# AntreasAntoniou/HowToTrainYourMAMLPytorch

Measured on AMD Instinct MI355X. Metric: meta-tasks/sec, higher is better.
Workload: dtype bf16; 1 GPU; model=maml++_miniimagenet_5w1s, global_batch=128, tasks_per_gpu=128, ways=5, shots=1, targets=15, filters=48, inner_steps=5, msl=True, parallelism=task-dp1

## Files before the change

howtotrainyourmamlpytorch_amd/ops/hip/dconv.hip:

```cpp

#include "common.h"
#include <torch/extension.h>
#include <ATen/cuda/CUDAContext.h>

using namespace maml355;

using bf16 = __hip_bfloat16;
typedef __attribute__((__vector_size__(8 * sizeof(short)))) short bf16x8;

template <int FT>
__global__ __launch_bounds__(256)
void dconv_fwd_kernel(const bf16* __restrict__ X, const float* __restrict__ W,
                      const float* __restrict__ bias, bf16* __restrict__ Y,
                      int T, int NB, int H, int Wd, int C,
                      int Ho, int Wo, int pad) {
  const int t = blockIdx.y;
  __shared__ float wl[9 * 8 * FT];
  const float* Wt = W + (long)t * FT * C * 9;
  for (int i = threadIdx.x; i < FT * C * 9; i += blockDim.x) {
    const int kyx = i % 9;
    const int c = (i / 9) % C;
    const int f = i / (9 * C);
    wl[(kyx * C + c) * FT + f] = Wt[i];
  }
  __syncthreads();

  const long Mtot = (long)NB * Ho * Wo;
  const bf16* Xt = X + (long)t * NB * H * Wd * C;
  bf16* Yt = Y + (long)t * Mtot * FT;
  const float* bt = bias ? bias + (long)t * FT : nullptr;

  for (long m = (long)blockIdx.x * blockDim.x + threadIdx.x; m < Mtot;
       m += (long)blockDim.x * gridDim.x) {
    const int wo = (int)(m % Wo);
    const int ho = (int)((m / Wo) % Ho);
    const int n = (int)(m / ((long)Wo * Ho));
    float acc[FT];
#pragma unroll
    for (int f = 0; f < FT; ++f) acc[f] = bt ? bt[f] : 0.f;
    for (int ky = 0; ky < 3; ++ky) {
      const int h = ho + ky - pad;
      if (h < 0 || h >= H) continue;
      for (int kx = 0; kx < 3; ++kx) {
        const int w = wo + kx - pad;
        if (w < 0 || w >= Wd) continue;
        const short* xrow = (const short*)Xt + (((long)n * H + h) * Wd + w) * C;
        for (int c = 0; c < C; ++c) {
          const float xv = __bfloat162float(
              __hip_bfloat16(__hip_bfloat16_raw{(unsigned short)xrow[c]}));
          const float* wp = &wl[((ky * 3 + kx) * C + c) * FT];
#pragma unroll
          for (int f = 0; f < FT; ++f) acc[f] = fmaf(xv, wp[f], acc[f]);
        }
      }
    }
#pragma unroll
    for (int f8 = 0; f8 < FT / 8; ++f8) {
      bf16x8 v;
#pragma unroll
      for (int j = 0; j < 8; ++j)
        v[j] = (short)__bfloat16_as_short(__float2bfloat16(acc[f8 * 8 + j]));
      *(bf16x8*)&((short*)Yt)[m * FT + f8 * 8] = v;
    }
  }
}

template <int CT, bool DET>
__global__ __launch_bounds__(256)
void dconv_wgrad_kernel(const bf16* __restrict__ dY, const bf16* __restrict__ X,
                        float* __restrict__ dWacc, float* __restrict__ dBacc,
                        int T, int NB, int H, int Wd, int Ho, int Wo, int F,
                        int pad, long chunk) {
  const int t = blockIdx.y;
  const long Mtot = (long)NB * Ho * Wo;
  const int wave = threadIdx.x / WAVE;
  const int lane = threadIdx.x % WAVE;
  const int nwaves = blockDim.x / WAVE;
  const long c0 = blockIdx.x * chunk + wave * (chunk / nwaves);
  const long c1 = min(c0 + chunk / nwaves, Mtot);

  const bf16* Xt = X + (long)t * NB * H * Wd * CT;
  const short* dYt = (const short*)dY + (long)t * Mtot * F;

  float acc[9 * CT];
#pragma unroll
  for (int i = 0; i < 9 * CT; ++i) acc[i] = 0.f;
  float db = 0.f;

  if (c0 < Mtot) {
    int wo = (int)(c0 % Wo);
    int ho = (int)((c0 / Wo) % Ho);
    int n = (int)(c0 / ((long)Wo * Ho));
    for (long m = c0; m < c1; ++m) {
      const float dyv =
          (lane < F)
              ? __bfloat162float(__hip_bfloat16(
                    __hip_bfloat16_raw{(unsigned short)dYt[m * F + lane]}))
              : 0.f;
      db += dyv;
#pragma unroll
      for (int ky = 0; ky < 3; ++ky) {
        const int h = ho + ky - pad;
        if (h < 0 || h >= H) continue;
#pragma unroll
        for (int kx = 0; kx < 3; ++kx) {
          const int w = wo + kx - pad;
          if (w < 0 || w >= Wd) continue;
          const short* xrow =
              (const short*)Xt + (((long)n * H + h) * Wd + w) * CT;
#pragma unroll
          for (int c = 0; c < CT; ++c) {
            const float xv = __bfloat162float(__hip_bfloat16(
                __hip_bfloat16_raw{(unsigned short)xrow[c]}));
            acc[(ky * 3 + kx) * CT + c] = fmaf(dyv, xv, acc[(ky * 3 + kx) * CT + c]);
          }
        }
      }
      if (++wo == Wo) {
        wo = 0;
        if (++ho == Ho) { ho = 0; ++n; }
      }
    }
  }

  float* dWt = DET ? dWacc + ((long)t * gridDim.x + blockIdx.x) * 9 * CT * F
                   : dWacc + (long)t * 9 * CT * F;
  {
    __shared__ float red[256];
#pragma unroll
    for (int i = 0; i < 9 * CT; ++i) {
      red[threadIdx.x] = acc[i];
      __syncthreads();
      if (wave == 0 && lane < F) {
        float s = 0.f;
        for (int wv = 0; wv < nwaves; ++wv) s += red[wv * WAVE + lane];
        if (DET) {
          dWt[(long)i * F + lane] = s;
        } else {
          atomicAdd(&dWt[(long)i * F + lane], s);
        }
      }
      __syncthreads();
    }
  }
  if (dBacc != nullptr) {
    __shared__ float dbl[256];
    dbl[threadIdx.x] = db;
    __syncthreads();
    if (wave == 0 && lane < F) {
      float s = 0.f;
      for (int wv = 0; wv < nwaves; ++wv) s += dbl[wv * WAVE + lane];
      if (DET) {
        dBacc[((long)t * gridDim.x + blockIdx.x) * F + lane] = s;
      } else {
        atomicAdd(&dBacc[(long)t * F + lane], s);
      }
    }
  }
}

__global__ void dconv_finalize_kernel(const float* __restrict__ acc,
                                      float* __restrict__ dw,
                                      int T, int F, int C, int nslices) {
  const long total = (long)T * F * C * 9;
  const long ssz = (long)9 * C * F;
  for (long i = (long)blockIdx.x * blockDim.x + threadIdx.x; i < total;
       i += grid_stride()) {
    long r = i;
    const int kx = (int)(r % 3); r /= 3;
    const int ky = (int)(r % 3); r /= 3;
    const int c = (int)(r % C); r /= C;
    const int f = (int)(r % F); r /= F;
    const long t = r;
    const long e = ((long)(ky * 3 + kx) * C + c) * F + f;
    float v = 0.f;
    for (int s = 0; s < nslices; ++s) v += acc[(t * nslices + s) * ssz + e];
    dw[i] = v;
  }
}

torch::Tensor dconv_fwd(torch::Tensor x, torch::Tensor w,
                        c10::optional<torch::Tensor> bias, long pad,
                        long Ho, long Wo) {
  TORCH_CHECK(x.is_cuda() && x.dim() == 5 && x.is_contiguous());
  TORCH_CHECK(x.scalar_type() == torch::kBFloat16);
  const int T = (int)x.size(0), NB = (int)x.size(1), H = (int)x.size(2),
            W = (int)x.size(3), C = (int)x.size(4);
  const int F = (int)w.size(1);
  TORCH_CHECK(C <= 8 && (F == 16 || F == 32 || F == 48 || F == 64),
              "dconv_fwd needs C<=8 and F in {16,32,48,64}");
  auto wc = w.contiguous().to(torch::kFloat32);
  auto y = torch::empty({T, NB, Ho, Wo, F}, x.options());
  const float* bptr = nullptr;
  torch::Tensor bc;
  if (bias.has_value()) {
    bc = bias->contiguous().to(torch::kFloat32);
    bptr = bc.data_ptr<float>();
  }
  const long Mtot = (long)NB * Ho * Wo;
  const int blocks = (int)std::min<long>((Mtot + 255) / 256, 4096);
  auto stream = at::cuda::getCurrentCUDAStream();
#define LAUNCH_DFWD(FT)                                                        \
  hipLaunchKernelGGL((dconv_fwd_kernel<FT>), dim3(blocks, T), dim3(256), 0,    \
                     stream.stream(),                                          \
                     reinterpret_cast<const bf16*>(x.data_ptr()),              \
                     wc.data_ptr<float>(), bptr,                               \
                     reinterpret_cast<bf16*>(y.data_ptr()),                    \
                     T, NB, H, W, C, (int)Ho, (int)Wo, (int)pad)
  switch (F) {
    case 16: LAUNCH_DFWD(16); break;
    case 32: LAUNCH_DFWD(32); break;
    case 48: LAUNCH_DFWD(48); break;
    default: LAUNCH_DFWD(64); break;
  }
#undef LAUNCH_DFWD
  return y;
}

std::vector<torch::Tensor> dconv_wgrad(torch::Tensor dy, torch::Tensor x,
                                       long pad, bool with_bias) {
  TORCH_CHECK(dy.is_cuda() && x.is_cuda());
  auto dyc = dy.contiguous();
  auto xc = x.contiguous();
  const int T = (int)x.size(0), NB = (int)x.size(1), H = (int)x.size(2),
            W = (int)x.size(3), C = (int)x.size(4);
  const int Ho = (int)dy.size(2), Wo = (int)dy.size(3), F = (int)dy.size(4);
  TORCH_CHECK(C <= 8 && F <= 64, "dconv_wgrad needs C<=8, F<=64");
  const char* det_env = getenv("MAML355_DETERMINISTIC");
  const bool det = det_env && det_env[0] == '1';
  const long Mtot = (long)NB * Ho * Wo;
  long gridx = std::max<long>(1, 2048 / std::max(1, T));
  long chunk = (Mtot + gridx - 1) / gridx;
  chunk = std::max<long>(((chunk + 3) / 4) * 4, 4);
  gridx = (Mtot + chunk - 1) / chunk;
  const int nslices = det ? (int)gridx : 1;
  auto acc = torch::zeros({T, nslices, 9 * C, F},
                          x.options().dtype(torch::kFloat32));
  auto dbacc = torch::zeros({T, nslices, F},
                            x.options().dtype(torch::kFloat32));
  auto stream = at::cuda::getCurrentCUDAStream();
#define LAUNCH_DWG(CT, DET_)                                                   \
  hipLaunchKernelGGL((dconv_wgrad_kernel<CT, DET_>), dim3((unsigned)gridx, T), \
                     dim3(256), 0, stream.stream(),                            \
                     reinterpret_cast<const bf16*>(dyc.data_ptr()),            \
                     reinterpret_cast<const bf16*>(xc.data_ptr()),             \
                     acc.data_ptr<float>(),                                    \
                     with_bias ? dbacc.data_ptr<float>() : nullptr,            \
                     T, NB, H, W, Ho, Wo, F, (int)pad, chunk)
#define LAUNCH_DWG_DET(CT)                                                     \
  do { if (det) LAUNCH_DWG(CT, true); else LAUNCH_DWG(CT, false); } while (0)
  switch (C) {
    case 1: LAUNCH_DWG_DET(1); break;
    case 2: LAUNCH_DWG_DET(2); break;
    case 3: LAUNCH_DWG_DET(3); break;
    case 4: LAUNCH_DWG_DET(4); break;
    default: LAUNCH_DWG_DET(8); break;
  }
#undef LAUNCH_DWG
#undef LAUNCH_DWG_DET
  auto dw = torch::empty({T, F, C, 3, 3}, x.options().dtype(torch::kFloat32));
  const long total = (long)T * F * C * 9;
  const int fb = (int)std::min<long>((total + 255) / 256, 4096);
  hipLaunchKernelGGL(dconv_finalize_kernel, dim3(fb), dim3(256), 0,
                     stream.stream(), acc.data_ptr<float>(),
                     dw.data_ptr<float>(), T, F, C, nslices);
  auto db = nslices == 1 ? dbacc.select(1, 0).contiguous() : dbacc.sum(1);
  return {dw, db};
}
```

howtotrainyourmamlpytorch_amd/ops/hip/tconv.hip:

```cpp

#include "common.h"
#include <torch/extension.h>
#include <ATen/cuda/CUDAContext.h>

using namespace maml355;

using bf16 = __hip_bfloat16;
typedef __attribute__((__vector_size__(8 * sizeof(short)))) short bf16x8;
typedef __attribute__((__vector_size__(4 * sizeof(float)))) float f32x4;

DEVINL int swz64(int row, int col) {
  return (row * 64 + col) ^ ((row & 7) << 3);
}
DEVINL int swz128(int row, int col) {
  return (row * 128 + col) ^ ((row & 7) << 3);
}

__global__ void repack_weight_kernel(const float* __restrict__ w,
                                     bf16* __restrict__ wp,
                                     int T, int F, int C, bool dgrad) {
  const long total = (long)T * F * C * 9;
  for (long i = (long)blockIdx.x * blockDim.x + threadIdx.x; i < total;
       i += grid_stride()) {
    long r = i;
    const int kx = (int)(r % 3); r /= 3;
    const int ky = (int)(r % 3); r /= 3;
    const int c = (int)(r % C); r /= C;
    const int f = (int)(r % F); r /= F;
    const long t = r;
    const float v = w[i];
    long o;
    if (!dgrad) {
      o = (((t * 9 + (long)(ky * 3 + kx)) * C + c) * F) + f;
    } else {
      o = (((t * 9 + (long)((2 - ky) * 3 + (2 - kx))) * F + f) * C) + c;
    }
    wp[o] = __float2bfloat16(v);
  }
}

__global__ void wgrad_finalize_kernel(const float* __restrict__ acc,
                                      float* __restrict__ dw,
                                      int T, int F, int C, int nslices) {
  const long total = (long)T * F * C * 9;
  const long ssz = (long)9 * C * F;
  for (long i = (long)blockIdx.x * blockDim.x + threadIdx.x; i < total;
       i += grid_stride()) {
    long r = i;
    const int kx = (int)(r % 3); r /= 3;
    const int ky = (int)(r % 3); r /= 3;
    const int c = (int)(r % C); r /= C;
    const int f = (int)(r % F); r /= F;
    const long t = r;
    const long e = ((long)(ky * 3 + kx) * C + c) * F + f;
    float v = 0.f;
    for (int s = 0; s < nslices; ++s) {
      v += acc[(t * nslices + s) * ssz + e];
    }
    dw[i] = v;
  }
}

#define BM 256
#define BK 64
#define WG_KCHUNK 4096
#define WBK 64

#define WGN 64

__global__ __launch_bounds__(512, 2)
void tconv_mm_kernel(const bf16* __restrict__ X, const bf16* __restrict__ Wp,
                     const float* __restrict__ bias, bf16* __restrict__ Y,
                     float* __restrict__ sums_out,
                     int T, int NB, int H, int W, int Ci,
                     int Ho, int Wo, int Co, int pad) {
  const int t = blockIdx.y;
  const long Mtot = (long)NB * Ho * Wo;
  const long m0 = (long)blockIdx.x * BM;
  const int K9 = 9 * Ci;
  const int ksteps = (K9 + BK - 1) / BK;
  const int ntiles = (Co + 15) / 16;

  __shared__ short lds_a[BM * BK];
  __shared__ short lds_bt[64 * BK];
// ... 80 lines not shown
        if (k0 + kk < K9) {
          v = *(const bf16x8*)&((const short*)Wt)[(long)(k0 + kk) * Co + f0];
        }
#pragma unroll
        for (int j = 0; j < 8; ++j)
          lds_bt[swz64(f0 + j, kk & ~7) + (kk & 7)] = v[j];
      } else {
        for (int j = 0; j < 8 && f0 + j < 64; ++j) {
          const int f = f0 + j;
          short v = 0;
          if (f < Co && k0 + kk < K9) {
            v = ((const short*)Wt)[(long)(k0 + kk) * Co + f];
          }
          lds_bt[swz64(f, kk & ~7) + (kk & 7)] = v;
        }
      }
    }
    __syncthreads();

#pragma unroll
    for (int ksl = 0; ksl < BK / 32; ++ksl) {
      bf16x8 a0 = *(const bf16x8*)&lds_a[swz64(wave * 32 + fr, ksl * 32 + fk * 8)];
      bf16x8 a1 = *(const bf16x8*)&lds_a[swz64(wave * 32 + 16 + fr, ksl * 32 + fk * 8)];
#pragma unroll
      for (int nt = 0; nt < 4; ++nt) {
        if (nt < ntiles) {
          bf16x8 b = *(const bf16x8*)&lds_bt[swz64(nt * 16 + fr, ksl * 32 + fk * 8)];
          acc[0][nt] = __builtin_amdgcn_mfma_f32_16x16x32_bf16(a0, b, acc[0][nt], 0, 0, 0);
          acc[1][nt] = __builtin_amdgcn_mfma_f32_16x16x32_bf16(a1, b, acc[1][nt], 0, 0, 0);
        }
      }
    }
    __syncthreads();
  }

  __shared__ float sums_lds[2][64];
  if (sums_out) {
    for (int i = threadIdx.x; i < 128; i += blockDim.x) {
      sums_lds[i >> 6][i & 63] = 0.f;
    }
    __syncthreads();
  }
  bf16* Yt = Y + (long)t * Mtot * Co;
#pragma unroll
  for (int hh = 0; hh < 2; ++hh)
#pragma unroll
  for (int nt = 0; nt < 4; ++nt) {
    if (nt >= ntiles) break;
    const int col = nt * 16 + fr;
    if (col >= Co) continue;
    const float bv = bias ? bias[(long)t * Co + col] : 0.f;
    float ls = 0.f, lq = 0.f;
#pragma unroll
    for (int j = 0; j < 4; ++j) {
      const int row = wave * 32 + hh * 16 + fk * 4 + j;
      const long mg = m0 + row;
      if (mg < Mtot) {
        const float v = acc[hh][nt][j] + bv;
        ((short*)Yt)[mg * Co + col] =
            (short)__bfloat16_as_short(__float2bfloat16(v));
        ls += v;
        lq += v * v;
      }
    }
    if (sums_out) {
      atomicAdd(&sums_lds[0][col], ls);
      atomicAdd(&sums_lds[1][col], lq);
    }
  }
  if (sums_out) {
    __syncthreads();
    for (int c = threadIdx.x; c < Co; c += blockDim.x) {
      atomicAdd(&sums_out[((long)t * 2 + 0) * Co + c], sums_lds[0][c]);
      atomicAdd(&sums_out[((long)t * 2 + 1) * Co + c], sums_lds[1][c]);
    }
  }
}

#define V2_LDS_BYTES (2 * BM * BK * 2 + 2 * 64 * BK * 2)
#define V2_LDS_BYTES_SBUF (BM * BK * 2 + 64 * BK * 2)

template <bool DBUF>
__global__ __launch_bounds__(512, 2)
void tconv_mm_v2_kernel(const bf16* __restrict__ Xp, const bf16* __restrict__ Wimg,
                        const float* __restrict__ bias, const bf16* __restrict__ zpage,
                        bf16* __restrict__ Y, float* __restrict__ sums_out,
                        int T, int NB, int Hp, int Wp, int Ci,
                        int Ho, int Wo, int Co) {
  const int t = blockIdx.y;
  const long Mtot = (long)NB * Ho * Wo;
  const long m0 = (long)blockIdx.x * BM;
  const int K9 = 9 * Ci;
  const int ksteps = (K9 + BK - 1) / BK;
  const int ntiles = (Co + 15) / 16;

  extern __shared__ short smem[];
#define LDS_A(buf_) (smem + (DBUF ? (buf_) * (BM * BK) : 0))
#define LDS_B(buf_) \
  (smem + (DBUF ? 2 : 1) * (BM * BK) + (DBUF ? (buf_) * (64 * BK) : 0))

  const bf16* Xt = Xp + (long)t * NB * Hp * Wp * Ci;
  const short* Wt = (const short*)Wimg + (long)t * ksteps * 64 * BK;

  const int wave = threadIdx.x / WAVE;
  const int lane = threadIdx.x % WAVE;
  const int fr = lane & 15;
  const int fk = lane >> 4;

  int a_rb[4];
  int a_c[4], a_dy[4], a_dx[4], a_koff[4], a_k[4];
#pragma unroll
  for (int q = 0; q < 4; ++q) {
    const int s = q * 512 + threadIdx.x;
    const int m = s >> 3;
    const int k8 = ((s & 7) ^ (m & 7)) * 8;
    a_k[q] = k8;
    const int kyx = k8 / Ci;
    a_c[q] = k8 - kyx * Ci;
    a_dy[q] = kyx / 3;
    a_dx[q] = kyx % 3;
    a_koff[q] = (a_dy[q] * Wp + a_dx[q]) * Ci + a_c[q];
    const long mg = m0 + m;
    if (mg < Mtot) {
      const int wo = (int)(mg % Wo);
      const int ho = (int)((mg / Wo) % Ho);
      const int n = (int)(mg / ((long)Wo * Ho));
      a_rb[q] = ((n * Hp + ho) * Wp + wo) * Ci;
    } else {
      a_rb[q] = -1;
    }
  }
#define V2_ADVANCE()                                                           \
  do {                                                                         \
    _Pragma("unroll")                                                          \
    for (int q = 0; q < 4; ++q) {                                              \
      a_k[q] += BK;                                                            \
      a_c[q] += BK;                                                            \
      while (a_c[q] >= Ci) {                                                   \
        a_c[q] -= Ci;                                                          \
        if (++a_dx[q] == 3) { a_dx[q] = 0; ++a_dy[q]; }                        \
      }                                                                        \
      a_koff[q] = (a_dy[q] * Wp + a_dx[q]) * Ci + a_c[q];                      \
    }                                                                          \
  } while (0)

#define V2_STAGE(ks_, buf_)                                                    \
  do {                                                                         \
    _Pragma("unroll")                                                          \
    for (int q = 0; q < 4; ++q) {                                              \
      const bf16* src = (a_rb[q] < 0 || a_k[q] >= K9)                          \
                            ? zpage                                            \
                            : Xt + a_rb[q] + a_koff[q];                        \
      auto ldst = (__attribute__((address_space(3))) void*)(                   \
          &LDS_A(buf_)[((long)q * 512 + wave * 64) * 8]);                      \
      __builtin_amdgcn_global_load_lds(                                        \
          (const __attribute__((address_space(1))) void*)src, ldst, 16, 0, 0); \
    }                                                                          \
    {                                                                          \
      const short* bsrc = Wt + (long)(ks_)*64 * BK + (long)threadIdx.x * 8;    \
      auto ldst = (__attribute__((address_space(3))) void*)(                   \
          &LDS_B(buf_)[(long)wave * 64 * 8]);                                  \
      __builtin_amdgcn_global_load_lds(                                        \
          (const __attribute__((address_space(1))) void*)bsrc, ldst, 16, 0, 0);\
    }                                                                          \
  } while (0)

  f32x4 acc[2][4];
#pragma unroll
  for (int hh = 0; hh < 2; ++hh)
#pragma unroll
    for (int i = 0; i < 4; ++i) acc[hh][i] = {0.f, 0.f, 0.f, 0.f};

  int buf = 0;
  if (DBUF) {
    V2_STAGE(0, 0);
    __syncthreads();
  }
  for (int ks = 0; ks < ksteps; ++ks) {
    if (DBUF) {
      V2_ADVANCE();
      if (ks + 1 < ksteps) V2_STAGE(ks + 1, buf ^ 1);
    } else {
      V2_STAGE(ks, 0);
      V2_ADVANCE();
      __syncthreads();
    }
    const short* la = LDS_A(buf);
    const short* lb = LDS_B(buf);
#pragma unroll
    for (int ksl = 0; ksl < BK / 32; ++ksl) {
      bf16x8 a0 = *(const bf16x8*)&la[swz64(wave * 32 + fr, ksl * 32 + fk * 8)];
      bf16x8 a1 = *(const bf16x8*)&la[swz64(wave * 32 + 16 + fr, ksl * 32 + fk * 8)];
#pragma unroll
      for (int nt = 0; nt < 4; ++nt) {
        if (nt < ntiles) {
          bf16x8 b = *(const bf16x8*)&lb[swz64(nt * 16 + fr, ksl * 32 + fk * 8)];
          acc[0][nt] = __builtin_amdgcn_mfma_f32_16x16x32_bf16(a0, b, acc[0][nt], 0, 0, 0);
          acc[1][nt] = __builtin_amdgcn_mfma_f32_16x16x32_bf16(a1, b, acc[1][nt], 0, 0, 0);
        }
      }
    }
    __syncthreads();
    if (DBUF) buf ^= 1;
  }
#undef V2_STAGE
#undef V2_ADVANCE

  __shared__ float sums_lds[2][64];
  if (sums_out) {
    for (int i = threadIdx.x; i < 128; i += blockDim.x) {
      sums_lds[i >> 6][i & 63] = 0.f;
    }
    __syncthreads();
  }
  bf16* Yt = Y + (long)t * Mtot * Co;
#pragma unroll
  for (int hh = 0; hh < 2; ++hh)
#pragma unroll
  for (int nt = 0; nt < 4; ++nt) {
    if (nt >= ntiles) break;
    const int col = nt * 16 + fr;
    if (col >= Co) continue;
    const float bv = bias ? bias[(long)t * Co + col] : 0.f;
    float ls = 0.f, lq = 0.f;
#pragma unroll
    for (int j = 0; j < 4; ++j) {
      const int row = wave * 32 + hh * 16 + fk * 4 + j;
      const long mg = m0 + row;
      if (mg < Mtot) {
        const float v = acc[hh][nt][j] + bv;
        ((short*)Yt)[mg * Co + col] =
            (short)__bfloat16_as_short(__float2bfloat16(v));
        ls += v;
        lq += v * v;
      }
// ... 467 lines not shown
      }
    }
    __syncthreads();

#pragma unroll
    for (int ks = 0; ks < WBK / 32; ++ks) {
      bf16x8 b = *(const bf16x8*)&lds_bt[swz64(wave * 16 + fr, ks * 32 + fk * 8)];
#pragma unroll
      for (int mt = 0; mt < 4; ++mt) {
        if (mt < mtiles) {
          bf16x8 a = *(const bf16x8*)&lds_at[swz64(mt * 16 + fr, ks * 32 + fk * 8)];
          acc[mt] = __builtin_amdgcn_mfma_f32_16x16x32_bf16(a, b, acc[mt], 0, 0, 0);
        }
      }
    }
    if (do_bias && db_f < F) {
#pragma unroll
      for (int kk = db_q * 16; kk < db_q * 16 + 16; ++kk) {
        db_acc += __bfloat162float(__hip_bfloat16(__hip_bfloat16_raw{
            (unsigned short)lds_at[swz64(db_f, kk & ~7) + (kk & 7)]}));
      }
    }
  }
  if (do_bias) {
    __shared__ float db_lds[4][64];
    db_lds[db_q][db_f] = db_acc;
    __syncthreads();
    if (db_q == 0 && db_f < F) {
      const float v = db_lds[0][db_f] + db_lds[1][db_f] + db_lds[2][db_f] +
                      db_lds[3][db_f];
      if (DET) {
        dBacc[((long)t * gridDim.y + blockIdx.y) * F + db_f] = v;
      } else {
        atomicAdd(&dBacc[(long)t * F + db_f], v);
      }
    }
  }

  float* dWt = DET ? dWacc + ((long)t * gridDim.y + blockIdx.y) * N9 * F
                   : dWacc + (long)t * N9 * F;
#pragma unroll
  for (int mt = 0; mt < 4; ++mt) {
    if (mt >= mtiles) break;
#pragma unroll
    for (int j = 0; j < 4; ++j) {
      const int f = mt * 16 + fk * 4 + j;
      const int n = n0 + wave * 16 + fr;
      if (f < F && n < N9) {
        if (DET) {
          dWt[(long)n * F + f] = acc[mt][j];
        } else {
          atomicAdd(&dWt[(long)n * F + f], acc[mt][j]);
        }
      }
    }
  }
}

__global__ void mfma_probe_kernel(const bf16* __restrict__ A,
                                  const bf16* __restrict__ B,
                                  float* __restrict__ D) {
  const int lane = threadIdx.x & (WAVE - 1);
  const int fr = lane & 15;
  const int fk = lane >> 4;
  bf16x8 a, b;
#pragma unroll
  for (int j = 0; j < 8; ++j) {
    a[j] = ((const short*)A)[fr * 32 + fk * 8 + j];
    b[j] = ((const short*)B)[(fk * 8 + j) * 16 + fr];
  }
  f32x4 d = {0.f, 0.f, 0.f, 0.f};
  d = __builtin_amdgcn_mfma_f32_16x16x32_bf16(a, b, d, 0, 0, 0);
#pragma unroll
  for (int j = 0; j < 4; ++j) {
    D[(fk * 4 + j) * 16 + fr] = d[j];
  }
}

namespace {
int ew_grid2(long total, int threads) {
  long blocks = (total + threads - 1) / threads;
  return (int)std::min<long>(blocks, 4096);
}
}

torch::Tensor tconv_repack(torch::Tensor w, bool dgrad) {
  TORCH_CHECK(w.is_cuda() && w.dim() == 5 && w.size(3) == 3 && w.size(4) == 3);
  auto wc = w.contiguous().to(torch::kFloat32);
  const int T = (int)w.size(0), F = (int)w.size(1), C = (int)w.size(2);
  auto wp = torch::empty({T, 9, dgrad ? F : C, dgrad ? C : F},
                         w.options().dtype(torch::kBFloat16));
  auto stream = at::cuda::getCurrentCUDAStream();
  const long total = (long)T * F * C * 9;
  hipLaunchKernelGGL(repack_weight_kernel, dim3(ew_grid2(total, 256)), dim3(256),
                     0, stream.stream(), wc.data_ptr<float>(),
                     reinterpret_cast<bf16*>(wp.data_ptr()), T, F, C, dgrad);
  return wp;
}

std::vector<torch::Tensor> tconv_mm(torch::Tensor x, torch::Tensor wp,
                                    c10::optional<torch::Tensor> bias, long pad,
                                    long Ho, long Wo, bool with_stats) {
  TORCH_CHECK(x.is_cuda() && x.dim() == 5 && x.is_contiguous());
  TORCH_CHECK(x.scalar_type() == torch::kBFloat16, "tconv_mm needs bf16");
  const int T = (int)x.size(0), NB = (int)x.size(1), H = (int)x.size(2),
            W = (int)x.size(3), Ci = (int)x.size(4);
  const int Co = (int)wp.size(3);
  TORCH_CHECK(wp.size(2) == Ci && Co <= 64, "Co must be <= 64");
  auto y = torch::empty({T, NB, Ho, Wo, Co}, x.options());
  auto sums = with_stats
                  ? torch::zeros({T, 2, Co}, x.options().dtype(torch::kFloat32))
                  : torch::empty({0}, x.options().dtype(torch::kFloat32));
  const long Mtot = (long)NB * Ho * Wo;
  dim3 grid((unsigned)((Mtot + BM - 1) / BM), T);
  auto stream = at::cuda::getCurrentCUDAStream();
  const int mm_threads = 512;
  const float* bptr = nullptr;
  torch::Tensor bc;
  if (bias.has_value()) {
    bc = bias->contiguous().to(torch::kFloat32);
    bptr = bc.data_ptr<float>();
  }
  hipLaunchKernelGGL(tconv_mm_kernel, grid, dim3(mm_threads), 0, stream.stream(),
                     reinterpret_cast<const bf16*>(x.data_ptr()),
                     reinterpret_cast<const bf16*>(wp.data_ptr()), bptr,
                     reinterpret_cast<bf16*>(y.data_ptr()),
                     with_stats ? sums.data_ptr<float>() : nullptr,
                     T, NB, H, W, Ci, (int)Ho, (int)Wo, Co, (int)pad);
  return {y, sums};
}

torch::Tensor tconv_repack_v2(torch::Tensor w, bool dgrad) {
  TORCH_CHECK(w.is_cuda() && w.dim() == 5 && w.size(3) == 3 && w.size(4) == 3);
  auto wc = w.contiguous().to(torch::kFloat32);
  const int T = (int)w.size(0), F = (int)w.size(1), C = (int)w.size(2);
  const int cin = dgrad ? F : C;
  const int ksteps = (9 * cin + BK - 1) / BK;
  auto out = torch::empty({T, ksteps, 64, BK},
                          w.options().dtype(torch::kBFloat16));
  auto stream = at::cuda::getCurrentCUDAStream();
  const long total = (long)T * ksteps * 64 * BK;
  hipLaunchKernelGGL(repack_v2_kernel, dim3(ew_grid2(total, 256)), dim3(256), 0,
                     stream.stream(), wc.data_ptr<float>(),
                     reinterpret_cast<bf16*>(out.data_ptr()), T, F, C, ksteps,
                     dgrad);
  return out;
}

std::vector<torch::Tensor> tconv_mm_v2(torch::Tensor x, torch::Tensor wimg,
                                       c10::optional<torch::Tensor> bias,
                                       long pad, long Ho, long Wo, long Co,
                                       bool with_stats) {
  TORCH_CHECK(x.is_cuda() && x.dim() == 5 && x.is_contiguous());
  TORCH_CHECK(x.scalar_type() == torch::kBFloat16, "tconv_mm_v2 needs bf16");
  const int T = (int)x.size(0), NB = (int)x.size(1), H = (int)x.size(2),
            W = (int)x.size(3), Ci = (int)x.size(4);
  TORCH_CHECK(Ci % 8 == 0 && Co <= 64);
  auto stream = at::cuda::getCurrentCUDAStream();
  torch::Tensor xp = x;
  int Hp = H, Wp = W;
  if (pad > 0) {
    Hp = H + 2 * (int)pad;
    Wp = W + 2 * (int)pad;
    xp = torch::empty({T, NB, Hp, Wp, Ci}, x.options());
    const long ptotal = (long)T * NB * Hp * Wp * (Ci / 8);
    hipLaunchKernelGGL(pad_nhwc_kernel, dim3(ew_grid2(ptotal, 256)), dim3(256),
                       0, stream.stream(),
                       reinterpret_cast<const bf16*>(x.data_ptr()),
                       reinterpret_cast<bf16*>(xp.data_ptr()),
                       T, NB, H, W, Ci, (int)pad);
  }
  auto y = torch::empty({T, NB, Ho, Wo, Co}, x.options());
  auto sums = with_stats
                  ? torch::zeros({T, 2, Co}, x.options().dtype(torch::kFloat32))
                  : torch::empty({0}, x.options().dtype(torch::kFloat32));
  auto zpage_cache = torch::zeros({16}, x.options());
  const float* bptr = nullptr;
  torch::Tensor bc;
  if (bias.has_value()) {
    bc = bias->contiguous().to(torch::kFloat32);
    bptr = bc.data_ptr<float>();
  }
  const long Mtot = (long)NB * Ho * Wo;
  dim3 grid((unsigned)((Mtot + BM - 1) / BM), T);
  const char* sbuf_env = getenv("MAML355_CONV_V2_SBUF");
  const bool sbuf = !(sbuf_env && sbuf_env[0] == '0');
  static bool attr_set = false;
  if (!attr_set) {
    hipFuncSetAttribute((const void*)tconv_mm_v2_kernel<true>,
                        hipFuncAttributeMaxDynamicSharedMemorySize,
                        V2_LDS_BYTES);
    hipFuncSetAttribute((const void*)tconv_mm_v2_kernel<false>,
                        hipFuncAttributeMaxDynamicSharedMemorySize,
                        V2_LDS_BYTES_SBUF);
    attr_set = true;
  }
#define LAUNCH_MMV2(DB_, BYTES_)                                               \
  hipLaunchKernelGGL((tconv_mm_v2_kernel<DB_>), grid, dim3(512), BYTES_,       \
                     stream.stream(),                                          \
                     reinterpret_cast<const bf16*>(xp.data_ptr()),             \
                     reinterpret_cast<const bf16*>(wimg.data_ptr()), bptr,     \
                     reinterpret_cast<const bf16*>(zpage_cache.data_ptr()),    \
                     reinterpret_cast<bf16*>(y.data_ptr()),                    \
                     with_stats ? sums.data_ptr<float>() : nullptr,            \
                     T, NB, Hp, Wp, Ci, (int)Ho, (int)Wo, (int)Co)
  if (sbuf) LAUNCH_MMV2(false, V2_LDS_BYTES_SBUF);
  else LAUNCH_MMV2(true, V2_LDS_BYTES);
#undef LAUNCH_MMV2
  return {y, sums};
}

std::vector<torch::Tensor> tconv_wgrad(torch::Tensor dy, torch::Tensor x,
                                       long pad, bool with_bias) {
  TORCH_CHECK(dy.is_cuda() && x.is_cuda());
  auto dyc = dy.contiguous();
  auto xc = x.contiguous();
  const int T = (int)x.size(0), NB = (int)x.size(1), H = (int)x.size(2),
            W = (int)x.size(3), C = (int)x.size(4);
  const int Ho = (int)dy.size(2), Wo = (int)dy.size(3), F = (int)dy.size(4);
  TORCH_CHECK(F <= 64, "F must be <= 64");
  const int N9 = 9 * C;
  const long Ktot = (long)NB * Ho * Wo;
  const char* det_env = getenv("MAML355_DETERMINISTIC");
  const bool det = det_env && det_env[0] == '1';
  const int gridx = (N9 + WGN - 1) / WGN;
  long desired_y = std::max<long>(1, 1024 / std::max<long>(1, (long)gridx * T));
  long kchunk = (Ktot + desired_y - 1) / desired_y;
  kchunk = ((kchunk + WBK - 1) / WBK) * WBK;
  kchunk = std::max<long>(kchunk, WBK);
  if (!det) kchunk = std::min<long>(kchunk, WG_KCHUNK);
  const int gridy = (int)((Ktot + kchunk - 1) / kchunk);
  const int nslices = det ? gridy : 1;
  auto acc = torch::zeros({T, nslices, N9, F},
                          x.options().dtype(torch::kFloat32));
  auto dbacc = torch::zeros({T, nslices, F},
                            x.options().dtype(torch::kFloat32));
  dim3 grid((unsigned)gridx, (unsigned)gridy, T);
  auto stream = at::cuda::getCurrentCUDAStream();
#define LAUNCH_WGRAD(DET_)                                                     \
  hipLaunchKernelGGL((tconv_wgrad_kernel<DET_>), grid, dim3(256), 0,           \
                     stream.stream(),                                          \
                     reinterpret_cast<const bf16*>(dyc.data_ptr()),            \
                     reinterpret_cast<const bf16*>(xc.data_ptr()),             \
                     acc.data_ptr<float>(),                                    \
                     with_bias ? dbacc.data_ptr<float>() : nullptr,            \
                     T, NB, H, W, C, Ho, Wo, F, (int)pad, (int)kchunk)
  if (det) LAUNCH_WGRAD(true); else LAUNCH_WGRAD(false);
#undef LAUNCH_WGRAD
  auto dw = torch::empty({T, F, C, 3, 3}, x.options().dtype(torch::kFloat32));
  const long total = (long)T * F * C * 9;
  hipLaunchKernelGGL(wgrad_finalize_kernel, dim3(ew_grid2(total, 256)),
                     dim3(256), 0, stream.stream(), acc.data_ptr<float>(),
                     dw.data_ptr<float>(), T, F, C, nslices);
  auto db = nslices == 1 ? dbacc.select(1, 0).contiguous() : dbacc.sum(1);
  return {dw, db};
}

std::vector<torch::Tensor> tconv_wgrad_v2(torch::Tensor dy, torch::Tensor x,
                                          long pad, bool with_bias) {
  TORCH_CHECK(dy.is_cuda() && x.is_cuda());
  auto dyc = dy.contiguous();
  auto xc = x.contiguous();
  const int T = (int)x.size(0), NB = (int)x.size(1), H = (int)x.size(2),
            W = (int)x.size(3), C = (int)x.size(4);
  const int Ho = (int)dy.size(2), Wo = (int)dy.size(3), F = (int)dy.size(4);
  TORCH_CHECK(F <= 64, "wgrad_v2 needs F <= 64");
  const char* det_env = getenv("MAML355_DETERMINISTIC");
  const bool det = det_env && det_env[0] == '1';
  const int N9 = 9 * C;
  const int Wo8 = ((Wo + 7) / 8) * 8;
  const long Kprime = (long)NB * Ho * Wo8;
  const long Kr = ((Kprime + WBK - 1) / WBK) * WBK;
  const int Hxp = H + 2 * (int)pad;
  const int Wxp = Wo8 + 2;
  auto stream = at::cuda::getCurrentCUDAStream();

  auto dyt = torch::empty({T, F, Kr}, x.options());
  {
    const long blocks = (long)T * NB * Ho;
    hipLaunchKernelGGL(dyt_pad_kernel, dim3((unsigned)blocks), dim3(256), 0,
                       stream.stream(),
                       reinterpret_cast<const bf16*>(dyc.data_ptr()),
                       reinterpret_cast<bf16*>(dyt.data_ptr()),
                       T, NB, Ho, Wo, F, Wo8, Kr);
    if (Kr > Kprime) {
      const long total = (long)T * F * (Kr - Kprime);
      hipLaunchKernelGGL(dyt_tail_kernel, dim3(ew_grid2(total, 256)), dim3(256),
                         0, stream.stream(),
                         reinterpret_cast<bf16*>(dyt.data_ptr()), T, F, Kprime,
                         Kr);
    }
  }
  auto xt = torch::empty({(long)T * C * NB * Hxp * Wxp}, x.options());
  {
    const long blocks = (long)T * NB * Hxp * ((Wxp + 63) / 64);
    hipLaunchKernelGGL(xt_pad_kernel, dim3((unsigned)blocks), dim3(256), 0,
                       stream.stream(),
                       reinterpret_cast<const bf16*>(xc.data_ptr()),
                       reinterpret_cast<bf16*>(xt.data_ptr()),
                       T, NB, H, W, C, Hxp, Wxp, (int)pad);
  }
  auto zpage = torch::zeros({16}, x.options());

  int nsub = (N9 > 64 && Kr >= 131072) ? 2 : 1;
  if (const char* e = getenv("MAML355_WGRAD_NSUB")) {
    if (e[0] == '1') nsub = 1; else if (e[0] == '2' && N9 > 64) nsub = 2;
  }
  const int wgn = 64 * nsub;

  const int gridx = (N9 + wgn - 1) / wgn;
  long desired_y = std::max<long>(1, 1024 / std::max<long>(1, (long)gridx * T));
  long kchunk = (Kr + desired_y - 1) / desired_y;
  kchunk = ((kchunk + WBK - 1) / WBK) * WBK;
  kchunk = std::max<long>(kchunk, WBK);
  if (!det) kchunk = std::min<long>(kchunk, (long)WG_KCHUNK);
  const int gridy = (int)((Kr + kchunk - 1) / kchunk);
  const int nslices = det ? gridy : 1;
  auto acc = torch::zeros({T, nslices, N9, F},
                          x.options().dtype(torch::kFloat32));
  auto dbacc = torch::zeros({T, nslices, F},
                            x.options().dtype(torch::kFloat32));
  dim3 grid((unsigned)gridx, (unsigned)gridy, T);
#define LAUNCH_WG2(NS_, DET_)                                                  \
  hipLaunchKernelGGL((tconv_wgrad_v2_kernel<NS_, DET_>), grid, dim3(256), 0,   \
                     stream.stream(),                                          \
                     reinterpret_cast<const bf16*>(dyt.data_ptr()),            \
                     reinterpret_cast<const bf16*>(xt.data_ptr()),             \
                     reinterpret_cast<const bf16*>(zpage.data_ptr()),          \
                     acc.data_ptr<float>(),                                    \
                     with_bias ? dbacc.data_ptr<float>() : nullptr,            \
                     T, NB, Ho, Wo8, Hxp, Wxp, C, F, Kr, Kprime, (int)kchunk)
  if (nsub == 2) {
    if (det) LAUNCH_WG2(2, true); else LAUNCH_WG2(2, false);
  } else {
    if (det) LAUNCH_WG2(1, true); else LAUNCH_WG2(1, false);
  }
#undef LAUNCH_WG2
  auto dw = torch::empty({T, F, C, 3, 3}, x.options().dtype(torch::kFloat32));
  const long total = (long)T * F * C * 9;
  hipLaunchKernelGGL(wgrad_finalize_kernel, dim3(ew_grid2(total, 256)),
                     dim3(256), 0, stream.stream(), acc.data_ptr<float>(),
                     dw.data_ptr<float>(), T, F, C, nslices);
  auto db = nslices == 1 ? dbacc.select(1, 0).contiguous() : dbacc.sum(1);
  return {dw, db};
}

void launch_wgrad_finalize(const float* acc, float* dw, int T, int F, int C,
                           int nslices, hipStream_t stream) {
  const long total = (long)T * F * C * 9;
  hipLaunchKernelGGL(wgrad_finalize_kernel, dim3(ew_grid2(total, 256)),
                     dim3(256), 0, stream, acc, dw, T, F, C, nslices);
}

std::vector<torch::Tensor> mfma_probe(torch::Tensor A, torch::Tensor B) {
  TORCH_CHECK(A.is_cuda() && A.sizes() == torch::IntArrayRef({16, 32}));
  TORCH_CHECK(B.sizes() == torch::IntArrayRef({32, 16}));
  auto Ac = A.contiguous().to(torch::kBFloat16);
  auto Bc = B.contiguous().to(torch::kBFloat16);
  auto D = torch::zeros({16, 16}, A.options().dtype(torch::kFloat32));
  auto stream = at::cuda::getCurrentCUDAStream();
  hipLaunchKernelGGL(mfma_probe_kernel, dim3(1), dim3(64), 0, stream.stream(),
                     reinterpret_cast<const bf16*>(Ac.data_ptr()),
                     reinterpret_cast<const bf16*>(Bc.data_ptr()),
                     D.data_ptr<float>());
  return {D};
}
```

Before: 606.1 tasks/s.

## Add MFMA first-layer conv, implicit padding in tconv, cached zero page

Adds a dconv forward v2 kernel for C=1 or 3. It keeps weights in registers, software-prefetches input pixels and computes with f32 16x16x4 MFMA instead of scalar FMAs over LDS. The tconv matmul kernel now does zero padding implicitly through bounds checks in new address helpers. This removes the separate padded copy of the input and its allocation. Per-call zero-page allocations are replaced by a per-device cached zero page. The costs are extra bounds-check logic in the load path and 32-bit offset limits, checked on the host.

Result: faster. 698.7 tasks/s, median of 6 (+15.3%).

```diff
diff --git a/howtotrainyourmamlpytorch_amd/ops/hip/dconv.hip b/howtotrainyourmamlpytorch_amd/ops/hip/dconv.hip
--- a/howtotrainyourmamlpytorch_amd/ops/hip/dconv.hip
+++ b/howtotrainyourmamlpytorch_amd/ops/hip/dconv.hip
@@ -63,6 +63,116 @@
       *(bf16x8*)&((short*)Yt)[m * FT + f8 * 8] = v;
     }
   }
+}
+
+typedef __attribute__((__vector_size__(4 * sizeof(float)))) float f32x4;
+typedef __attribute__((__vector_size__(4 * sizeof(short)))) short bf16x4;
+
+template <int FT, int CT>
+__global__ __launch_bounds__(256)
+void dconv_fwd_v2_kernel(const bf16* __restrict__ X, const float* __restrict__ W,
+                         const float* __restrict__ bias, bf16* __restrict__ Y,
+                         int NB, int H, int Wd, int Ho, int Wo, int pad) {
+  constexpr int K = 9 * CT;
+  constexpr int KS = (K + 3) / 4;
+  constexpr int NT = FT / 16;
+  constexpr int kInvalid = -(1 << 30);
+  const int t = blockIdx.y;
+  const int wave = __builtin_amdgcn_readfirstlane(threadIdx.x / WAVE);
+  const int lane = threadIdx.x % WAVE;
+  const int li = lane & 15;
+  const int g = lane >> 4;
+  const int Mtot = NB * Ho * Wo;
+  const int ntiles = (Mtot + 15) / 16;
+
+  const float* Wt = W + (long)t * FT * CT * 9;
+  const unsigned short* Xt =
+      (const unsigned short*)X + (long)t * NB * H * Wd * CT;
+  short* Yt = (short*)Y + (long)t * Mtot * FT;
+
+  float wa[KS][NT];
+  int koff[KS], kdy[KS], kdx[KS];
+#pragma unroll
+  for (int s = 0; s < KS; ++s) {
+    const int k = 4 * s + g;
+    const bool kv = k < K;
+    const int tap = kv ? k / CT : 0;
+    const int c = kv ? k - tap * CT : 0;
+    const int dy = tap / 3, dx = tap - dy * 3;
+#pragma unroll
+    for (int nt = 0; nt < NT; ++nt)
+      wa[s][nt] = kv ? Wt[((nt * 16 + li) * CT + c) * 9 + tap] : 0.f;
+    koff[s] = (dy * Wd + dx) * CT + c;
+    kdy[s] = kv ? dy : (1 << 20);
+    kdx[s] = dx;
+  }
+  f32x4 bv[NT];
+#pragma unroll
+  for (int nt = 0; nt < NT; ++nt)
+#pragma unroll
+    for (int j = 0; j < 4; ++j)
+      bv[nt][j] = bias ? bias[(long)t * FT + nt * 16 + g * 4 + j] : 0.f;
+
+  const int stride = gridDim.x * (blockDim.x / WAVE);
+  const int dm = stride * 16;
+  const int dwo = dm % Wo;
+  const int dho = (dm / Wo) % Ho;
+  const int dimg = (dm / Wo) / Ho;
+  int tile = blockIdx.x * (blockDim.x / WAVE) + wave;
+  int m = tile * 16 + li;
+  int wo = m % Wo, ho = (m / Wo) % Ho, img = (m / Wo) / Ho;
+
+  unsigned short xr[KS];
+#define DFWD2_LOAD()                                                           \
+  do {                                                                         \
+    const bool mv = m < Mtot;                                                  \
+    const int hb = mv ? ho - pad : kInvalid;                                   \
+    const int wb = wo - pad;                                                   \
+    const int base = mv ? ((img * H + hb) * Wd + wb) * CT : 0;                 \
+    _Pragma("unroll")                                                          \
+    for (int s = 0; s < KS; ++s) {                                             \
+      const bool ok = (unsigned)(hb + kdy[s]) < (unsigned)H &&                 \
+                      (unsigned)(wb + kdx[s]) < (unsigned)Wd;                  \
+      xr[s] = ok ? Xt[base + koff[s]] : (unsigned short)0;                     \
+    }                                                                          \
+  } while (0)
+
+  DFWD2_LOAD();
+  for (; tile < ntiles; tile += stride) {
+    float xb[KS];
+#pragma unroll
+    for (int s = 0; s < KS; ++s)
+      xb[s] = __uint_as_float((unsigned)xr[s] << 16);
+    const int m_cur = m;
+    m += dm;
+    wo += dwo;
+    if (wo >= Wo) { wo -= Wo; ho += 1; }
+    ho += dho;
+    if (ho >= Ho) { ho -= Ho; img += 1; }
+    img += dimg;
+    DFWD2_LOAD();
+
+    f32x4 acc[NT];
+#pragma unroll
+    for (int nt = 0; nt < NT; ++nt) acc[nt] = bv[nt];
+#pragma unroll
+    for (int s = 0; s < KS; ++s)
+#pragma unroll
+      for (int nt = 0; nt < NT; ++nt)
+        acc[nt] = __builtin_amdgcn_mfma_f32_16x16x4f32(wa[s][nt], xb[s],
+                                                       acc[nt], 0, 0, 0);
+    if (m_cur < Mtot) {
+#pragma unroll
+      for (int nt = 0; nt < NT; ++nt) {
+        bf16x4 v;
+#pragma unroll
+        for (int j = 0; j < 4; ++j)
+          v[j] = (short)__bfloat16_as_short(__float2bfloat16(acc[nt][j]));
+        *(bf16x4*)&Yt[(long)m_cur * FT + nt * 16 + g * 4] = v;
+      }
+    }
+  }
+#undef DFWD2_LOAD
 }
 
 template <int CT, bool DET>
@@ -198,9 +308,39 @@
     bptr = bc.data_ptr<float>();
   }
   const long Mtot = (long)NB * Ho * Wo;
+  auto stream = at::cuda::getCurrentCUDAStream();
+  const char* v2_env = getenv("MAML355_DCONV_FWD_V2");
+  const bool v2 = (C == 1 || C == 3) && !(v2_env && v2_env[0] == '0');
+  if (v2) {
+    TORCH_CHECK(Ho == H + 2 * pad - 2 && Wo == W + 2 * pad - 2 && Ho >= 1 &&
+                    Wo >= 1 && pad >= 0,
+                "dconv_fwd: Ho/Wo do not match a stride-1 3x3 conv");
+    TORCH_CHECK(Mtot < (1L << 30) && (long)NB * H * W * C < (1L << 30),
+                "dconv_fwd: task too large for 32-bit offsets");
+    const long ntiles = (Mtot + 15) / 16;
+    const int blocks2 =
+        (int)std::max<long>(1, std::min<long>((ntiles + 31) / 32, 2048));
+#define LAUNCH_DFWD2(FT, CT)                                                   \
+  hipLaunchKernelGGL((dconv_fwd_v2_kernel<FT, CT>), dim3(blocks2, T),          \
+                     dim3(256), 0, stream.stream(),                            \
+                     reinterpret_cast<const bf16*>(x.data_ptr()),              \
+                     wc.data_ptr<float>(), bptr,                               \
+                     reinterpret_cast<bf16*>(y.data_ptr()),                    \
+                     NB, H, W, (int)Ho, (int)Wo, (int)pad)
+#define LAUNCH_DFWD2_C(FT)                                                     \
+  do { if (C == 1) LAUNCH_DFWD2(FT, 1); else LAUNCH_DFWD2(FT, 3); } while (0)
+    switch (F) {
+      case 16: LAUNCH_DFWD2_C(16); break;
+      case 32: LAUNCH_DFWD2_C(32); break;
+      case 48: LAUNCH_DFWD2_C(48); break;
+      default: LAUNCH_DFWD2_C(64); break;
+    }
+#undef LAUNCH_DFWD2_C
+#undef LAUNCH_DFWD2
+    return y;
+  }
   const int blocks = (int)std::min<long>((Mtot + 255) / 256, 4096);
-  auto stream = at::cuda::getCurrentCUDAStream();
-#define LAUNCH_DFWD(FT)                                                        \
+#define LAUNCH_DFWD(FT)                                                       \
   hipLaunchKernelGGL((dconv_fwd_kernel<FT>), dim3(blocks, T), dim3(256), 0,    \
                      stream.stream(),                                          \
                      reinterpret_cast<const bf16*>(x.data_ptr()),              \
diff --git a/howtotrainyourmamlpytorch_amd/ops/hip/tconv.hip b/howtotrainyourmamlpytorch_amd/ops/hip/tconv.hip
--- a/howtotrainyourmamlpytorch_amd/ops/hip/tconv.hip
+++ b/howtotrainyourmamlpytorch_amd/ops/hip/tconv.hip
@@ -1,5 +1,6 @@
 
 #include "common.h"
+#include "tconv_mm_addr.h"
 #include <torch/extension.h>
 #include <ATen/cuda/CUDAContext.h>
 
@@ -246,13 +247,14 @@
 
 template <bool DBUF>
 __global__ __launch_bounds__(512, 2)
-void tconv_mm_v2_kernel(const bf16* __restrict__ Xp, const bf16* __restrict__ Wimg,
+void tconv_mm_v2_kernel(const bf16* __restrict__ X, const bf16* __restrict__ Wimg,
                         const float* __restrict__ bias, const bf16* __restrict__ zpage,
                         bf16* __restrict__ Y, float* __restrict__ sums_out,
-                        int T, int NB, int Hp, int Wp, int Ci,
-                        int Ho, int Wo, int Co) {
+                        int T, int NB, int H, int W, int Ci,
+                        int Ho, int Wo, int Co, int pad) {
   const int t = blockIdx.y;
-  const long Mtot = (long)NB * Ho * Wo;
+  const tcmm::Geom g = tcmm::make_geom(NB, H, W, Ci, Ho, Wo, pad);
+  const long Mtot = g.Mtot;
   const long m0 = (long)blockIdx.x * BM;
   const int K9 = 9 * Ci;
   const int ksteps = (K9 + BK - 1) / BK;
@@ -263,7 +265,7 @@
 #define LDS_B(buf_) \
   (smem + (DBUF ? 2 : 1) * (BM * BK) + (DBUF ? (buf_) * (64 * BK) : 0))
 
-  const bf16* Xt = Xp + (long)t * NB * Hp * Wp * Ci;
+  const bf16* Xt = X + (long)t * NB * H * W * Ci;
   const short* Wt = (const short*)Wimg + (long)t * ksteps * 64 * BK;
 
   const int wave = threadIdx.x / WAVE;
@@ -271,50 +273,21 @@
   const int fr = lane & 15;
   const int fk = lane >> 4;
 
-  int a_rb[4];
-  int a_c[4], a_dy[4], a_dx[4], a_koff[4], a_k[4];
+  tcmm::KState a_k = tcmm::k_init(g, tcmm::slot_k8(threadIdx.x));
+  tcmm::Row a_row[4];
 #pragma unroll
   for (int q = 0; q < 4; ++q) {
-    const int s = q * 512 + threadIdx.x;
-    const int m = s >> 3;
-    const int k8 = ((s & 7) ^ (m & 7)) * 8;
-    a_k[q] = k8;
-    const int kyx = k8 / Ci;
-    a_c[q] = k8 - kyx * Ci;
-    a_dy[q] = kyx / 3;
-    a_dx[q] = kyx % 3;
-    a_koff[q] = (a_dy[q] * Wp + a_dx[q]) * Ci + a_c[q];
-    const long mg = m0 + m;
-    if (mg < Mtot) {
-      const int wo = (int)(mg % Wo);
-      const int ho = (int)((mg / Wo) % Ho);
-      const int n = (int)(mg / ((long)Wo * Ho));
-      a_rb[q] = ((n * Hp + ho) * Wp + wo) * Ci;
-    } else {
-      a_rb[q] = -1;
-    }
-  }
-#define V2_ADVANCE()                                                           \
-  do {                                                                         \
-    _Pragma("unroll")                                                          \
-    for (int q = 0; q < 4; ++q) {                                              \
-      a_k[q] += BK;                                                            \
-      a_c[q] += BK;                                                            \
-      while (a_c[q] >= Ci) {                                                   \
-        a_c[q] -= Ci;                                                          \
-        if (++a_dx[q] == 3) { a_dx[q] = 0; ++a_dy[q]; }                        \
-      }                                                                        \
-      a_koff[q] = (a_dy[q] * Wp + a_dx[q]) * Ci + a_c[q];                      \
-    }                                                                          \
-  } while (0)
+    a_row[q] = tcmm::row_init(g, m0 + tcmm::slot_row(q * 512 + threadIdx.x));
+  }
+#define V2_ADVANCE() tcmm::k_advance(g, a_k)
 
 #define V2_STAGE(ks_, buf_)                                                    \
   do {                                                                         \
     _Pragma("unroll")                                                          \
     for (int q = 0; q < 4; ++q) {                                              \
-      const bf16* src = (a_rb[q] < 0 || a_k[q] >= K9)                          \
-                            ? zpage                                            \
-                            : Xt + a_rb[q] + a_koff[q];                        \
+      int off;                                                                 \
+      const bf16* src = tcmm::slot_src(g, a_row[q], a_k, off) ? Xt + off       \
+                                                              : zpage;         \
       auto ldst = (__attribute__((address_space(3))) void*)(                   \
           &LDS_A(buf_)[((long)q * 512 + wave * 64) * 8]);                      \
       __builtin_amdgcn_global_load_lds(                                        \
@@ -948,6 +921,15 @@
   long blocks = (total + threads - 1) / threads;
   return (int)std::min<long>(blocks, 4096);
 }
+
+const bf16* conv_zero_page(const torch::Tensor& like) {
+  static auto* pages = new std::vector<torch::Tensor>(64);
+  const int dev = like.get_device();
+  TORCH_CHECK(dev >= 0 && dev < 64);
+  auto& p = (*pages)[dev];
+  if (!p.defined()) p = torch::zeros({128}, like.options());
+  return reinterpret_cast<const bf16*>(p.data_ptr());
+}
 }
 
 torch::Tensor tconv_repack(torch::Tensor w, bool dgrad) {
@@ -1022,10 +1004,18 @@
   const int T = (int)x.size(0), NB = (int)x.size(1), H = (int)x.size(2),
             W = (int)x.size(3), Ci = (int)x.size(4);
   TORCH_CHECK(Ci % 8 == 0 && Co <= 64);
+  TORCH_CHECK(pad >= 0 && pad <= 2 && Ho == H + 2 * pad - 2 &&
+              Wo == W + 2 * pad - 2 && Ho >= 1 && Wo >= 1,
+              "tconv_mm_v2: Ho/Wo do not match a stride-1 3x3 conv");
+  TORCH_CHECK((long)NB * (H + 4) * (W + 4) * Ci < (1L << 31),
+              "tconv_mm_v2: task too large for 32-bit offsets");
   auto stream = at::cuda::getCurrentCUDAStream();
+  const char* nopad_env = getenv("MAML355_CONV_V2_NOPAD");
+  const bool nopad = !(nopad_env && nopad_env[0] == '0');
   torch::Tensor xp = x;
-  int Hp = H, Wp = W;
-  if (pad > 0) {
+  int Hp = H, Wp = W, kpad = (int)pad;
+  if (!nopad && pad > 0) {
+    kpad = 0;
     Hp = H + 2 * (int)pad;
     Wp = W + 2 * (int)pad;
     xp = torch::empty({T, NB, Hp, Wp, Ci}, x.options());
@@ -1040,7 +1030,11 @@
   auto sums = with_stats
                   ? torch::zeros({T, 2, Co}, x.options().dtype(torch::kFloat32))
                   : torch::empty({0}, x.options().dtype(torch::kFloat32));
-  auto zpage_cache = torch::zeros({16}, x.options());
+  torch::Tensor zpage_call;
+  if (!nopad) zpage_call = torch::zeros({16}, x.options());
+  const bf16* zpage =
+      nopad ? conv_zero_page(x)
+            : reinterpret_cast<const bf16*>(zpage_call.data_ptr());
   const float* bptr = nullptr;
   torch::Tensor bc;
   if (bias.has_value()) {
@@ -1066,10 +1060,9 @@
                      stream.stream(),                                          \
                      reinterpret_cast<const bf16*>(xp.data_ptr()),             \
                      reinterpret_cast<const bf16*>(wimg.data_ptr()), bptr,     \
-                     reinterpret_cast<const bf16*>(zpage_cache.data_ptr()),    \
-                     reinterpret_cast<bf16*>(y.data_ptr()),                    \
+                     zpage, reinterpret_cast<bf16*>(y.data_ptr()),             \
                      with_stats ? sums.data_ptr<float>() : nullptr,            \
-                     T, NB, Hp, Wp, Ci, (int)Ho, (int)Wo, (int)Co)
+                     T, NB, Hp, Wp, Ci, (int)Ho, (int)Wo, (int)Co, kpad)
   if (sbuf) LAUNCH_MMV2(false, V2_LDS_BYTES_SBUF);
   else LAUNCH_MMV2(true, V2_LDS_BYTES);
 #undef LAUNCH_MMV2
@@ -1166,7 +1159,7 @@
                        reinterpret_cast<bf16*>(xt.data_ptr()),
                        T, NB, H, W, C, Hxp, Wxp, (int)pad);
   }
-  auto zpage = torch::zeros({16}, x.options());
+  const bf16* zpage = conv_zero_page(x);
 
   int nsub = (N9 > 64 && Kr >= 131072) ? 2 : 1;
   if (const char* e = getenv("MAML355_WGRAD_NSUB")) {
@@ -1191,8 +1184,7 @@
   hipLaunchKernelGGL((tconv_wgrad_v2_kernel<NS_, DET_>), grid, dim3(256), 0,   \
                      stream.stream(),                                          \
                      reinterpret_cast<const bf16*>(dyt.data_ptr()),            \
-                     reinterpret_cast<const bf16*>(xt.data_ptr()),             \
-                     reinterpret_cast<const bf16*>(zpage.data_ptr()),          \
+                     reinterpret_cast<const bf16*>(xt.data_ptr()), zpage,      \
                      acc.data_ptr<float>(),                                    \
                      with_bias ? dbacc.data_ptr<float>() : nullptr,            \
                      T, NB, Ho, Wo8, Hxp, Wxp, C, F, Kr, Kprime, (int)kchunk)
diff --git a/howtotrainyourmamlpytorch_amd/ops/hip/tconv_mm_addr.h b/howtotrainyourmamlpytorch_amd/ops/hip/tconv_mm_addr.h
--- /dev/null
+++ b/howtotrainyourmamlpytorch_amd/ops/hip/tconv_mm_addr.h
@@ -0,0 +1,83 @@
+#pragma once
+
+#if defined(__HIPCC__) || defined(__CUDACC__)
+#define TCMM_HD __host__ __device__ inline
+#else
+#define TCMM_HD inline
+#endif
+
+namespace maml355 {
+namespace tcmm {
+
+constexpr int kBM = 256;
+constexpr int kBK = 64;
+constexpr int kThreads = 512;
+constexpr int kSlotsPerThread = 4;
+
+struct Geom {
+  int NB, H, W, Ci;
+  int Ho, Wo, pad;
+  long Mtot;
+  int K9;
+};
+
+TCMM_HD Geom make_geom(int NB, int H, int W, int Ci, int Ho, int Wo, int pad) {
+  Geom g;
+  g.NB = NB; g.H = H; g.W = W; g.Ci = Ci;
+  g.Ho = Ho; g.Wo = Wo; g.pad = pad;
+  g.Mtot = (long)NB * Ho * Wo;
+  g.K9 = 9 * Ci;
+  return g;
+}
+
+TCMM_HD int slot_row(int s) { return s >> 3; }
+TCMM_HD int slot_k8(int s) { return ((s & 7) ^ ((s >> 3) & 7)) * 8; }
+
+struct KState { int c, dy, dx; };
+
+TCMM_HD KState k_init(const Geom& g, int k8) {
+  KState s;
+  const int tap = k8 / g.Ci;
+  s.c = k8 - tap * g.Ci;
+  s.dy = tap / 3;
+  s.dx = tap - s.dy * 3;
+  return s;
+}
+
+TCMM_HD void k_advance(const Geom& g, KState& s) {
+  s.c += kBK;
+  while (s.c >= g.Ci) {
+    s.c -= g.Ci;
+    if (++s.dx == 3) { s.dx = 0; ++s.dy; }
+  }
+}
+
+struct Row { int rb, hb, wb; };
+
+constexpr int kRowInvalid = -(1 << 30);
+
+TCMM_HD Row row_init(const Geom& g, long mg) {
+  Row r;
+  if (mg < g.Mtot) {
+    const int wo = (int)(mg % g.Wo);
+    const int ho = (int)((mg / g.Wo) % g.Ho);
+    const int img = (int)(mg / ((long)g.Wo * g.Ho));
+    r.hb = ho - g.pad;
+    r.wb = wo - g.pad;
+    r.rb = ((img * g.H + r.hb) * g.W + r.wb) * g.Ci;
+  } else {
+    r.hb = kRowInvalid;
+    r.wb = 0;
+    r.rb = 0;
+  }
+  return r;
+}
+
+TCMM_HD bool slot_src(const Geom& g, const Row& r, const KState& k, int& off) {
+  off = r.rb + (k.dy * g.W + k.dx) * g.Ci + k.c;
+  return k.dy < 3 && (unsigned)(r.hb + k.dy) < (unsigned)g.H &&
+         (unsigned)(r.wb + k.dx) < (unsigned)g.W;
+}
+
+}
+}
```
